# GlassyWing/yolo_deepsort

Measured on AMD Instinct MI355X. Metric: end-to-end frames/sec (detect+ReID+assoc), 608x608, higher is better.
Workload: dtype f16x3

## Files before the change

### yolo_deepsort_amd/csrc/common.h

```cpp
#pragma once
#include <hip/hip_runtime.h>
#include <stdint.h>
#include <stdio.h>
#include <string>
#include <vector>
#include <stdexcept>

namespace yds {

void set_error(const std::string &msg);
struct Error : std::runtime_error {
    explicit Error(const std::string &m) : std::runtime_error(m) {}
};
[[noreturn]] void fail(const char *fmt, ...);
int bound_device();
void bind_thread();
hipStream_t make_stream(bool latency_role);

#define YDS_HIP(expr)                                                                          \
    do {                                                                                       \
        hipError_t _e = (expr);                                                                \
        if (_e != hipSuccess)                                                                  \
            ::yds::fail("%s failed: %s (%s:%d)", #expr, hipGetErrorString(_e), __FILE__, __LINE__); \
    } while (0)

#define YDS_API_BEGIN try { ::yds::bind_thread();
#define YDS_API_END                                                                            \
    }                                                                                          \
    catch (const std::exception &e) {                                                          \
        ::yds::set_error(e.what());                                                            \
        return -1;                                                                             \
    }                                                                                          \
    return 0;
#define YDS_API_END_PTR                                                                        \
    }                                                                                          \
    catch (const std::exception &e) {                                                          \
        ::yds::set_error(e.what());                                                            \
        return nullptr;                                                                        \
    }

template <typename T> struct DevBuf {
    T *p = nullptr;
    size_t n = 0;
    DevBuf() = default;
    explicit DevBuf(size_t count) { alloc(count); }
    DevBuf(const DevBuf &) = delete;
    DevBuf &operator=(const DevBuf &) = delete;
    DevBuf(DevBuf &&o) noexcept : p(o.p), n(o.n) { o.p = nullptr; o.n = 0; }
    DevBuf &operator=(DevBuf &&o) noexcept {
        if (this != &o) { release(); p = o.p; n = o.n; o.p = nullptr; o.n = 0; }
        return *this;
    }
    ~DevBuf() { release(); }
    void alloc(size_t count) {
        release();
        if (count == 0) return;
        YDS_HIP(hipMalloc((void **)&p, count * sizeof(T)));
        n = count;
    }
    void ensure(size_t count) { if (count > n) alloc(count); }
    void release() { if (p) { (void)hipFree(p); p = nullptr; n = 0; } }
    void upload(const T *src, size_t count, hipStream_t s = nullptr) {
        ensure(count);
        if (count) YDS_HIP(hipMemcpyAsync(p, src, count * sizeof(T), hipMemcpyHostToDevice, s));
    }
};

struct View {
    float *p = nullptr;
    int n = 0, h = 0, w = 0, c = 0, ld = 0;
    int fmt = 0;
    size_t pixels() const { return (size_t)n * h * w; }
};

enum Act { ACT_LINEAR = 0, ACT_LEAKY = 1, ACT_MISH = 2, ACT_RELU = 3 };
enum ResMode { RES_NONE = 0, RES_AFTER_ACT = 1, RES_BEFORE_ACT = 2 };

struct ConvArgs {
    View x, y;
    const float *w = nullptr, *bias = nullptr;
    const void *w16 = nullptr;
    View res;
    int ksize = 1, stride = 1, pad = 0, kpad = 0;
    int act = ACT_LINEAR, res_mode = RES_NONE;
    int terms = 3;
    View y2;
    int n_split = 0;
    int tile_gn = 0;
};
enum ConvVariant {
    VAR_F32_128x128_K32, VAR_F32_128x64_K32, VAR_F32_64x64_K32, VAR_F32_128x32_K32, VAR_F32_128x128_K16, VAR_F32_128x64_K16, VAR_F32_64x128_K16,
    VAR_STAGED_128x128, VAR_STAGED_64x128, VAR_STAGED_128x64, VAR_STAGED_64x64,
    VAR_DMA_128x128_NS2, VAR_DMA_256x128_NS3, VAR_DMA_128x256_NS3, VAR_DMA_128x128_NS3, VAR_WIN_256x128, VAR_WIN_256x64, VAR_WIN_128x64,
    VAR_DMA_128x64_NS2, VAR_DMA_64x128_NS2, VAR_WIN2_128x128, VAR_SPLITK_64x128, VAR_SPLITK_128x128, VAR_DIRECT_RGB, kConvVariants
};
static_assert(VAR_STAGED_128x128 == 7 && VAR_WIN_256x128 == 15 && VAR_SPLITK_64x128 == 21 && kConvVariants == 24, "variant ids are fixed");
int launch_conv(const ConvArgs &a, hipStream_t s, int variant = -1);
constexpr int kVariantMask = 0xff, kTileGnShift = 8;
bool conv_presplit_input(const ConvArgs &a);
bool launch_conv_maxpool3s2(const ConvArgs &a, hipStream_t s);
int conv_autotune(const ConvArgs &a, hipStream_t s, float *best_us);
std::vector<int> conv_candidates(const ConvArgs &a);
enum ConvMath { MATH_F32 = 0, MATH_F16X3 = 1 };
int conv_math();
void set_conv_math(int m);
void pack_weights_f16x3(const float *w, int cout, int kpad, std::vector<uint16_t> &out);
const char *conv_variant_name(int v);
double conv_flops(const ConvArgs &a);
double conv_bytes_io(const View &v);
double conv_bytes(const ConvArgs &a);

void launch_maxpool(const View &x, const View &y, int k, int stride, int pad, bool zero_pad_br, hipStream_t s);
void launch_upsample(const View &x, const View &y, int stride, hipStream_t s);
void launch_copy(const View &x, const View &y, hipStream_t s);
void launch_add(const View &a, const View &b, const View &y, hipStream_t s);
void launch_nchw_to_nhwc(const float *src_nchw, const View &y, int c_src, hipStream_t s);
void launch_nhwc_to_nchw(const View &x, float *dst_nchw, hipStream_t s);
void launch_pack_h16(const float *src_f32, const View &y, hipStream_t s);
void launch_yolo_decode(const View &head, float *out, int total_boxes, int box_off, int num_classes,
                        const float *anchors_wh , int A, int img_h, int img_w, hipStream_t s);
void launch_inject(const View &head, int image, const float *rows_dev, int n, int head_index, int num_classes,
                   float logit, hipStream_t s);
void launch_inject_batch(const View &head, int batch, const float *table_dev, const int *offsets_dev, int max_rows, int head_index,
                         int num_classes, float logit, hipStream_t s);
void launch_resize_u8(const uint8_t *frames, int n, int h, int w, const View &y, hipStream_t s, bool bgr = false);
void launch_window_resize(const uint8_t *frames, int h, int w, const int *tiles_dev, int T, int slot0, int n, const View &y, hipStream_t s,
                          bool bgr);
void launch_window_boxes(const float *pred, int n_boxes, int attrs, const int *tiles_dev, const float *scale_dev, int T, int slot0, int n,
                         float *dst, hipStream_t s);
void launch_crop_resize(const uint8_t *frames, int h, int w, const int *boxes5_dev, int D, const View &y,
                        hipStream_t s, bool bgr = false);
void launch_avgpool_l2norm(const View &x, float *out, hipStream_t s);

}
```

### yolo_deepsort_amd/csrc/conv.hip

```cpp
#include "conv_common.h"

#include <vector>

#include <map>
#include <string>
#include <string.h>

namespace yds {

template <int BM, int BN, int WM, int WN, int BK, int ACT, int RES>
__global__ __launch_bounds__(256, 2) void conv_igemm_f32(ConvKernelArgs p) {
    fp16_saturate_on();
    static_assert(WM * WN == 4, "4 waves per workgroup");
    static_assert(BK == 16 || BK == 32, "K step");
    constexpr int LDS_LD = BK + 4;
    constexpr int CPR = BK / 4;
    constexpr int RPP = 256 / CPR;
    constexpr int TM = BM / WM / 32, TN = BN / WN / 32;
    constexpr int A_ROWS = BM / RPP, B_ROWS = BN / RPP;
    static_assert(A_ROWS >= 1 && B_ROWS >= 1, "tile too small for the staging pattern");
    extern __shared__ __attribute__((aligned(16))) float smem[];
    float *As = smem;
    float *Bs = smem + 2 * BM * LDS_LD;

// ... 255 lines not shown
    c.y.h = a.x.h; c.y.w = a.x.w;
    ConvKernelArgs k = make_conv_args(c);
    if (!conv_pool_applicable(k)) return false;
    launch_conv_pool(k, s);
    return true;
}

static int g_math = -1;
int conv_math() {
    if (g_math < 0) {
        const char *e = getenv("YDS_CONV_MATH");
        g_math = (e && !strcmp(e, "f32")) ? MATH_F32 : MATH_F16X3;
    }
    return g_math;
}
void set_conv_math(int m) { g_math = m == MATH_F32 ? MATH_F32 : MATH_F16X3; }

enum ConvArith { ARITH_F32 = MATH_F32, ARITH_F16X3 = MATH_F16X3, ARITH_DIRECT };
struct ConvVariantInfo {
    const char *name;
    int arith;
    void (*launch)(ConvKernelArgs k, int tile, hipStream_t s);
    int tile;
    bool (*runs)(const ConvArgs &a, const ConvKernelArgs &k);
    bool (*timed)(const ConvArgs &a);
};

static void launch_f32(ConvKernelArgs k, int tile, hipStream_t s) {
    switch (tile) {
        case 0: launch_cfg<128, 128, 2, 2, 32>(k, s); break;
        case 1: launch_cfg<128, 64, 2, 2, 32>(k, s); break;
        case 2: launch_cfg<64, 64, 2, 2, 32>(k, s); break;
        case 3: launch_cfg<128, 32, 4, 1, 32>(k, s); break;
        case 4: launch_cfg<128, 128, 2, 2, 16>(k, s); break;
        case 5: launch_cfg<128, 64, 2, 2, 16>(k, s); break;
        default: launch_cfg<64, 128, 2, 2, 16>(k, s); break;
    }
}
static void launch_win2(ConvKernelArgs k, int, hipStream_t s) { launch_conv_win2(k, s); }
static void launch_direct(ConvKernelArgs k, int, hipStream_t s) {
    if (!conv_direct_applicable(k)) fail("conv: the direct RGB kernel does not apply to this layer");
    launch_conv_direct(k, s);
}

static bool runs_not_f16(const ConvArgs &a, const ConvKernelArgs &) { return a.x.fmt != FMT_F16; }
static bool runs_presplit(const ConvArgs &a, const ConvKernelArgs &) { return conv_presplit_input(a); }
static bool runs_win(const ConvArgs &a, const ConvKernelArgs &k) { return conv_presplit_input(a) && conv_win_applicable(k); }
static bool runs_win_small(const ConvArgs &a, const ConvKernelArgs &k) { return runs_win(a, k) && a.terms != 1 && conv_win16_small_applicable(k); }
static bool runs_win2(const ConvArgs &a, const ConvKernelArgs &k) { return conv_presplit_input(a) && conv_win2_applicable(k); }
template <int TILE> static bool runs_splitk(const ConvArgs &a, const ConvKernelArgs &k) { return conv_presplit_input(a) && conv_splitk_applicable(k, TILE); }
static bool runs_direct(const ConvArgs &, const ConvKernelArgs &k) { return conv_direct_applicable(k); }

static bool timed_always(const ConvArgs &) { return true; }
static bool timed_narrow(const ConvArgs &a) { return a.y.c <= 64; }
static bool timed_wide(const ConvArgs &a) { return a.y.c >= 128; }
static bool timed_never(const ConvArgs &) { return false; }
static bool timed_unmerged(const ConvArgs &a) { return !a.n_split; }

static const ConvVariantInfo kVariants[kConvVariants] = {
     {"conv_igemm_f32<128,128,2,2,32>", ARITH_F32, launch_f32, 0, runs_not_f16, timed_always},
     {"conv_igemm_f32<128,64,2,2,32>", ARITH_F32, launch_f32, 1, runs_not_f16, timed_always},
     {"conv_igemm_f32<64,64,2,2,32>", ARITH_F32, launch_f32, 2, runs_not_f16, timed_always},
     {"conv_igemm_f32<128,32,4,1,32>", ARITH_F32, launch_f32, 3, runs_not_f16, timed_narrow},
     {"conv_igemm_f32<128,128,2,2,16>", ARITH_F32, launch_f32, 4, runs_not_f16, timed_always},
     {"conv_igemm_f32<128,64,2,2,16>", ARITH_F32, launch_f32, 5, runs_not_f16, timed_always},
     {"conv_igemm_f32<64,128,2,2,16>", ARITH_F32, launch_f32, 6, runs_not_f16, timed_always},
     {"conv_igemm_f16x3<128,128>", ARITH_F16X3, launch_conv_f16x3_staged, 0, runs_not_f16, timed_always},
     {"conv_igemm_f16x3<64,128>", ARITH_F16X3, launch_conv_f16x3_staged, 1, runs_not_f16, timed_always},
     {"conv_igemm_f16x3<128,64>", ARITH_F16X3, launch_conv_f16x3_staged, 2, runs_not_f16, timed_always},
     {"conv_igemm_f16x3<64,64>", ARITH_F16X3, launch_conv_f16x3_staged, 3, runs_not_f16, timed_always},
     {"conv_igemm_f16x3_dma<128,128,2x2,2>", ARITH_F16X3, launch_conv_f16x3_dma, 0, runs_presplit, timed_always},
     {"conv_igemm_f16x3_dma<256,128,4x2,3>", ARITH_F16X3, launch_conv_f16x3_dma, 1, runs_presplit, timed_always},
     {"conv_igemm_f16x3_dma<128,256,2x4,3>", ARITH_F16X3, launch_conv_f16x3_dma, 2, runs_presplit, timed_always},
     {"conv_igemm_f16x3_dma<128,128,2x2,3>", ARITH_F16X3, launch_conv_f16x3_dma, 3, runs_presplit, timed_always},
     {"conv3x3_f16x3_win<256,128,4x2>", ARITH_F16X3, launch_conv_f16x3_win, 0, runs_win, timed_always},
     {"conv3x3_f16x3_win<256,64,8x1>", ARITH_F16X3, launch_conv_f16x3_win, 1, runs_win, timed_narrow},
     {"conv3x3_f16x3_win<128,64,4x1>", ARITH_F16X3, launch_conv_f16x3_win, 2, runs_win_small, timed_narrow},
     {"conv_igemm_f16x3_dma<128,64,2x2,2>", ARITH_F16X3, launch_conv_f16x3_dma, 4, runs_presplit, timed_always},
     {"conv_igemm_f16x3_dma<64,128,2x2,2>", ARITH_F16X3, launch_conv_f16x3_dma, 5, runs_presplit, timed_always},
     {"conv3x3_f16x3_win2<128,128,2x2>", ARITH_F16X3, launch_win2, 0, runs_win2, timed_wide},
     {"conv_igemm_f16x3_dma<64,128,2x2,2>+splitK", ARITH_F16X3, launch_conv_f16x3_splitk, 0, runs_splitk<0>, timed_never},
     {"conv_igemm_f16x3_dma<128,128,2x2,2>+splitK", ARITH_F16X3, launch_conv_f16x3_splitk, 1, runs_splitk<1>, timed_never},
     {"conv3x3_rgb_direct", ARITH_DIRECT, launch_direct, 0, runs_direct, timed_unmerged},
};

const char *conv_variant_name(int v) {
    if (v >= 0) v &= kVariantMask;
    return v >= 0 && v < kConvVariants ? kVariants[v].name : "?";
}

int launch_conv(const ConvArgs &a, hipStream_t s, int variant) {
    ConvKernelArgs k = make_conv_args(a);
    if (variant >= 0) {
        k.gn_req = std::max(a.tile_gn, (variant >> kTileGnShift) & 0xff);
        variant &= kVariantMask;
    } else {
        k.gn_req = a.tile_gn;
    }
    if (variant < 0 || variant >= kConvVariants) variant = conv_default_variant(a);
    const ConvVariantInfo &e = kVariants[variant];
    if (e.arith == ARITH_F32 && (k.fmt_x != FMT_F32 || k.fmt_y != FMT_F32 || k.fmt_r != FMT_F32))
        fail("conv: the fp32 MFMA kernel takes fp32 tensors only");
    if (e.arith == ARITH_F16X3) {
        if (!a.w16) fail("conv: f16x3 variant requested but the layer has no split weights");
        k.w = reinterpret_cast<const float *>(a.w16);
    }
    e.launch(k, e.tile, s);
    return variant;
}

std::vector<int> conv_candidates(const ConvArgs &a) {
    const ConvKernelArgs k = make_conv_args(a);
    std::vector<int> cand;
    for (int v = 0; v < kConvVariants; ++v) {
        const ConvVariantInfo &e = kVariants[v];
        if ((e.arith == conv_math() || e.arith == ARITH_DIRECT) && e.runs(a, k) && e.timed(a)) cand.push_back(v);
    }
    return cand;
}

static int conv_autotune_measured(const ConvArgs &a, hipStream_t s, float *best_us);

static std::map<std::string, int> &tune_cache() {
    static std::map<std::string, int> cache;
    static bool loaded = false;
    if (!loaded) {
        loaded = true;
        if (const char *path = getenv("YDS_TUNE_CACHE")) {
            if (FILE *f = fopen(path, "r")) {
                char key[256];
                int v;
                while (fscanf(f, "%255s %d", key, &v) == 2) cache[key] = v;
                fclose(f);
            }
        }
    }
    return cache;
}
static std::string tune_key(const ConvArgs &a) {
    char buf[256];
    int n = a.x.n;
    if (n > 64) {
        int p2 = 64;
        while (p2 * 2 <= n) p2 *= 2;
        n = n >= p2 + p2 / 2 ? p2 + p2 / 2 : p2;
    }
    snprintf(buf, sizeof buf, "m%d_n%d_h%d_w%d_c%d_ld%d_o%d_ho%d_wo%d_k%d_s%d_a%d_r%d_fx%d_fy%d_sp%d", conv_math() + (a.terms == 1 ? 10 : 0), n, a.x.h, a.x.w, a.x.c, a.x.ld, a.y.c,
             a.y.h, a.y.w, a.ksize, a.stride, a.act, a.res.p ? a.res_mode : 0, a.x.fmt, a.y.fmt, a.n_split);
    return buf;
}

int conv_autotune(const ConvArgs &a, hipStream_t s, float *best_us) {
    if (getenv("YDS_NO_AUTOTUNE")) return -1;
    if (const char *f = getenv("YDS_CONV_FORCE")) {
        const int v = atoi(f);
        if (v >= 0 && v < kConvVariants && kVariants[v].runs(a, make_conv_args(a))) return v;
        return conv_autotune_measured(a, s, best_us);
    }
    if (conv_math() == MATH_F16X3 && a.w16 && a.terms != 1 && a.n_split == 0 && conv_splitk_preferred(make_conv_args(a))) return VAR_SPLITK_64x128;
    const std::string key = tune_key(a);
    auto &cache = tune_cache();
    auto it = cache.find(key);
    if (it != cache.end()) return it->second;
    int v = conv_autotune_measured(a, s, best_us);
    cache[key] = v;
    if (const char *path = getenv("YDS_TUNE_CACHE")) {
// ... 51 lines not shown
```

### yolo_deepsort_amd/csrc/conv_common.h

```cpp
#pragma once
#include "common.h"
#include "h16.h"

#include <algorithm>
#include <stdlib.h>
#include <type_traits>

namespace yds {

typedef float f32x16 __attribute__((ext_vector_type(16)));
typedef float f32x4 __attribute__((ext_vector_type(4)));

typedef _Float16 h8 __attribute__((ext_vector_type(8)));
typedef _Float16 h4 __attribute__((ext_vector_type(4)));
constexpr float A_SCALE = 1.f / 256.f, LO_SCALE = 2048.f;
typedef __attribute__((address_space(3))) void lds_void_t;
typedef __attribute__((address_space(1))) const void glb_void_t;
template <int N> __device__ __forceinline__ void wait_vmcnt() { asm volatile("s_waitcnt vmcnt(%0)" ::"n"(N) : "memory"); }

struct ConvKernelArgs {
    const float *x, *w, *bias, *res;
    float *y;
    int H, W, Cin, ldx;
    int Ho, Wo, Cout, ldy, ldr;
    int ksize, stride, pad;
    int K, Kpad, M;
    int act, res_mode;
    int fmt_x, fmt_y, fmt_r;
    int terms;
    int ksplit = 1;
    float *y2 = nullptr;
    int ldy2 = 0, n_split = 0;
    int tiles_m, tiles_n, xm, rm, rn;
    int gn = 1;
    int gn_req = 0;
};

constexpr int KALIGN = 32;
constexpr int STAGGER = 24;

template <int ACT> __device__ __forceinline__ float apply_act(float v) {
    if (ACT == ACT_LEAKY) return v > 0.f ? v : v * 0.1f;
    if (ACT == ACT_RELU) return v > 0.f ? v : 0.f;
    if (ACT == ACT_MISH) {
        const float e = __builtin_amdgcn_exp2f(fminf(v, 20.f) * 1.44269504088896341f);
        const float n = e * (e + 2.f);
        const float m = v * (n * __builtin_amdgcn_rcpf(n + 2.f));
        return v > 20.f ? v : m;
    }
    return v;
}

__device__ __forceinline__ bool tile_of_block(const ConvKernelArgs &p, int &tm, int &tn) {
    const int b = blockIdx.x, xcd = b & 7, idx = b >> 3;
    int lm, ln;
    if (p.gn <= 1) {
        lm = idx % p.rm;
        ln = idx / p.rm;
    } else {
        const int per = p.rm * p.gn, grp = idx / per, w = idx - grp * per;
        const int g = min(p.gn, p.rn - grp * p.gn);
        lm = w / g;
        ln = grp * p.gn + (w - lm * g);
    }
    tm = (xcd % p.xm) * p.rm + lm;
    tn = (xcd / p.xm) * p.rn + ln;
    return tm < p.tiles_m && tn < p.tiles_n;
}

inline int plan_tile_map(ConvKernelArgs &k, int BM, int BN) {
    k.tiles_m = (k.M + BM - 1) / BM;
    k.tiles_n = (k.Cout + BN - 1) / BN;
    long best = -1;
    for (int xm = 1; xm <= 8; xm *= 2) {
        int xn = 8 / xm;
        int rm = (k.tiles_m + xm - 1) / xm, rn = (k.tiles_n + xn - 1) / xn;
        long waste = (long)rm * rn * 8 - (long)k.tiles_m * k.tiles_n;
        long cost = ((long)rm * BM + (long)rn * BN) * 64 + waste * (BM + BN);
        if (best < 0 || cost < best) { best = cost; k.xm = xm; k.rm = rm; k.rn = rn; }
    }
    k.gn = std::max(1, std::min(k.gn_req, k.rn));
    return 8 * k.rm * k.rn;
}

struct FlatRows {
    int m0;
    __device__ __forceinline__ int operator()(int row) const { return m0 + row; }
};
template <int BM, int BN, int WM, int WN, int ACT, int RES, int NT, class RowMap, bool ONE_PASS, class Store>
__device__ __forceinline__ void conv_epilogue_core(const ConvKernelArgs &p, Store store, float *stage, RowMap rows, int n0, int tid) {
    constexpr int ROWS = BM / WM, LD = BN + 4, C4 = BN / 4;
    constexpr int RSTEP = NT / C4;
    static_assert(NT % C4 == 0 && C4 % 2 == 0 && ROWS % RSTEP == 0, "tile width must divide the workgroup; lane pairs share a row");
    const int wave = tid >> 6, wm = wave / WN;
    const int c4 = tid % C4, rr = tid / C4;
    const int n = n0 + c4 * 4;
    const bool n_vec = n + 3 < p.Cout;
    const bool second = p.n_split > 0 && n >= p.n_split;
    float *const y_base = second ? p.y2 : p.y;
    const int y_ld = second ? p.ldy2 : p.ldy, ny = second ? n - p.n_split : n;
    float4 bias4 = make_float4(0.f, 0.f, 0.f, 0.f);
    if (n_vec) bias4 = *reinterpret_cast<const float4 *>(p.bias + n);
    else {
        if (n < p.Cout) bias4.x = p.bias[n];
        if (n + 1 < p.Cout) bias4.y = p.bias[n + 1];
        if (n + 2 < p.Cout) bias4.z = p.bias[n + 2];
    }
    constexpr int PER_PASS = ROWS / RSTEP, NRES = RES != RES_NONE ? WM * PER_PASS : 1;
    auto sweep = [&](auto yf_c, auto rf_c) {
        constexpr int YF = decltype(yf_c)::value, RF = decltype(rf_c)::value;
        constexpr bool YH = YF == FMT_H16, RH = RF == FMT_H16, YS = YF == FMT_F16, RS = RF == FMT_F16;
        float4 rraw[NRES];
        if (RES != RES_NONE) {
#pragma unroll
            for (int q = 0; q < NRES; ++q) {
                const int m = rows((q / PER_PASS) * ROWS + rr + (q % PER_PASS) * RSTEP);
                rraw[q] = make_float4(0.f, 0.f, 0.f, 0.f);
                if (m >= 0 && m < p.M && n < p.Cout) {
                    const float *rp = p.res + (size_t)m * p.ldr;
                    if (RH) {
                        const char *g = reinterpret_cast<const char *>(rp + (n & ~31)) + (n & 31) * 2;
                        const float2 hi = *reinterpret_cast<const float2 *>(g), lo = *reinterpret_cast<const float2 *>(g + 64);
                        rraw[q] = make_float4(hi.x, hi.y, lo.x, lo.y);
                    } else if (RS) {
                        const float2 h = *reinterpret_cast<const float2 *>(reinterpret_cast<const char *>(rp) + n * 2);
                        rraw[q] = make_float4(h.x, h.y, 0.f, 0.f);
                    } else if (n_vec) {
                        rraw[q] = *reinterpret_cast<const float4 *>(rp + n);
                    } else {
                        rraw[q].x = rp[n];
                        if (n + 1 < p.Cout) rraw[q].y = rp[n + 1];
                        if (n + 2 < p.Cout) rraw[q].z = rp[n + 2];
                    }
                }
            }
        }
#pragma unroll
        for (int pass = 0; pass < WM; ++pass) {
            if (ONE_PASS ? pass == 0 : wm == pass) store(stage + (ONE_PASS ? wm * ROWS * LD : 0));
            if (!ONE_PASS || pass == 0) __syncthreads();
#pragma unroll
            for (int k2 = 0; k2 < PER_PASS; ++k2) {
                const int r = rr + k2 * RSTEP;
                const int m = rows(pass * ROWS + r);
                const bool live = m >= 0 && m < p.M && n < p.Cout;
                float4 v = *reinterpret_cast<const float4 *>(stage + (ONE_PASS ? pass * ROWS * LD : 0) + r * LD + c4 * 4);
                float rs[4] = {0.f, 0.f, 0.f, 0.f};
                if (RES != RES_NONE) {
                    const float4 t = rraw[RES != RES_NONE ? pass * PER_PASS + k2 : 0];
                    if (RH) {
                        union { float2 f; h16x4 h; } uh, ul;
// ... 170 lines not shown
```

### yolo_deepsort_amd/csrc/conv_f16x3.hip

```cpp
#include "conv_common.h"

#include <map>
#include <mutex>

#include <math.h>
#include <string.h>

namespace yds {


constexpr int ROWB = 144;
__device__ __forceinline__ void split4(const f32x4 &v, h4 &hi, h4 &lo) {
#pragma unroll
    for (int c = 0; c < 4; ++c) {
        float xs = v[c] * A_SCALE;
        _Float16 h = (_Float16)xs;
        hi[c] = h;
        lo[c] = (_Float16)((xs - (float)h) * LO_SCALE);
    }
}

template <int BM, int BN, int ACT, int RES, int AIN>
__global__ __launch_bounds__(256, 2) void conv_igemm_f16x3(ConvKernelArgs p) {
    fp16_saturate_on();
// ... 421 lines not shown
    else for (int k = 0; k < 4; ++k) if (n + k < p.Cout) yp[n + k] = v[k];
}

int conv_splitk_factor(const ConvKernelArgs &k, int BM, int BN) {
    const long tiles = (long)((k.M + BM - 1) / BM) * ((k.Cout + BN - 1) / BN);
    const int nk = k.K / 32;
    int s = (int)((512 + tiles - 1) / tiles);
    s = std::min(s, std::min(16, nk / 4));
    return s >= 2 ? s : 1;
}

static float *splitk_workspace(size_t floats, hipStream_t s) {
    static std::mutex mu;
    static std::map<hipStream_t, DevBuf<float>> bufs;
    std::lock_guard<std::mutex> lock(mu);
    DevBuf<float> &b = bufs[s];
    if (b.n < floats) {
        YDS_HIP(hipStreamSynchronize(s));
        b.alloc(floats + floats / 2);
    }
    return b.p;
}

template <int BM, int BN> static void launch_splitk(const ConvKernelArgs &k, hipStream_t s) {
    if (k.fmt_x != FMT_H16 || k.Cin % 32) fail("conv: the split-K LDS-DMA kernel needs a pre-split (H16) input");
    if ((size_t)k.Cout * 4 > (size_t)ZERO_PAGE_BYTES) fail("conv: %d filters exceed the zero page used as the split-K bias", k.Cout);
    const int ksplit = conv_splitk_factor(k, BM, BN);
    if (ksplit < 2) fail("conv: split-K does not apply (the layer already has enough tiles or too few K steps)");
    const int ldw = (k.Cout + 3) / 4 * 4;
    float *ws = splitk_workspace((size_t)ksplit * k.M * ldw, s);
    ConvKernelArgs part = k;
    part.y = ws; part.ldy = ldw; part.fmt_y = FMT_F32;
    part.bias = reinterpret_cast<const float *>(zero_page_dev());
    part.res = nullptr; part.res_mode = RES_NONE; part.fmt_r = FMT_F32; part.act = ACT_LINEAR;
    part.ksplit = ksplit;
    launch_cfg_dma<BM, BN, 2, 2, 2>(part, s);
    const int c4 = (k.Cout + 3) / 4;
    hipLaunchKernelGGL(splitk_reduce_kernel, dim3(((size_t)k.M * c4 + 255) / 256), dim3(256), 0, s, ws, ksplit, k.M, ldw, k);
    YDS_HIP(hipGetLastError());
}

bool conv_splitk_preferred(const ConvKernelArgs &k) {
    if (k.fmt_x != FMT_H16 || k.Cin % 32) return false;
    const long tiles = (long)((k.M + 63) / 64) * ((k.Cout + 127) / 128);
    return tiles <= 128 && k.K / 32 >= 32 && conv_splitk_factor(k, 64, 128) >= 2;
}

bool conv_splitk_applicable(const ConvKernelArgs &k, int tile) {
    if (k.fmt_x != FMT_H16 || k.Cin % 32) return false;
    return tile == 0 ? conv_splitk_factor(k, 64, 128) >= 2 : conv_splitk_factor(k, 128, 128) >= 2;
}

template <int BM, int BN> static void launch_cfg16(const ConvKernelArgs &k, hipStream_t s) {
    if (k.fmt_x == FMT_F16) fail("conv: the register-staged kernel does not read 2-byte (F16) activations");
    constexpr size_t smem = 2ull * (BM + BN) * ROWB;
    dispatch_act_res(k, [&](auto A, auto R) {
        if (k.fmt_x == FMT_H16) launch_conv_tiles<conv_igemm_f16x3<BM, BN, A, R, FMT_H16>>(k, BM, BN, 1, 256, smem, s);
        else launch_conv_tiles<conv_igemm_f16x3<BM, BN, A, R, FMT_F32>>(k, BM, BN, 1, 256, smem, s);
    });
}

void launch_conv_f16x3_staged(ConvKernelArgs k, int tile, hipStream_t s) {
    switch (tile) {
        case 0: launch_cfg16<128, 128>(k, s); break;
        case 1: launch_cfg16<64, 128>(k, s); break;
        case 2: launch_cfg16<128, 64>(k, s); break;
        default: launch_cfg16<64, 64>(k, s); break;
    }
}

void launch_conv_f16x3_dma(ConvKernelArgs k, int tile, hipStream_t s) {
    switch (tile) {
        case 0: launch_cfg_dma<128, 128, 2, 2, 2>(k, s); break;
        case 1: launch_cfg_dma<256, 128, 4, 2, 3>(k, s); break;
        case 2: launch_cfg_dma<128, 256, 2, 4, 3>(k, s); break;
        case 3: launch_cfg_dma<128, 128, 2, 2, 3>(k, s); break;
        case 4: launch_cfg_dma<128, 64, 2, 2, 2>(k, s); break;
        default: launch_cfg_dma<64, 128, 2, 2, 2>(k, s); break;
    }
}

void launch_conv_f16x3_win(ConvKernelArgs k, int tile, hipStream_t s) {
    if (!conv_win_applicable(k)) fail("conv: the window-resident kernel needs a 3x3 stride-1 layer with a pre-split input and W <= 95 (W <= 318 for 32 input channels)");
    if (k.terms == 1) launch_conv_win(k, tile, s);
    else launch_conv_win16(k, tile, s);
}

void launch_conv_f16x3_splitk(ConvKernelArgs k, int tile, hipStream_t s) {
    if (tile == 0) launch_splitk<64, 128>(k, s);
    else launch_splitk<128, 128>(k, s);
}

void pack_weights_f16x3(const float *w, int cout, int kpad, std::vector<uint16_t> &out) {
    out.assign((size_t)cout * kpad * 2, 0);
    for (int o = 0; o < cout; ++o)
        for (int k = 0; k < kpad; ++k) {
            float x = w[(size_t)o * kpad + k];
            if (!(fabsf(x) < 65504.f)) fail("conv: weight %g does not fit the fp16 split (|w| must be < 65504)", (double)x);
            _Float16 h = (_Float16)x;
            _Float16 l = (_Float16)((x - (float)h) * LO_SCALE);
            size_t base = ((size_t)o * (kpad / 32) + k / 32) * 64;
            uint16_t hb, lb;
            memcpy(&hb, &h, 2);
            memcpy(&lb, &l, 2);
            out[base + (k & 31)] = hb;
            out[base + 32 + (k & 31)] = lb;
        }
}

}
```

### yolo_deepsort_amd/csrc/conv_win16.hip

```cpp
#include "conv_win_common.h"

namespace yds {
namespace {

template <int BM, int BN, int WM, int WN, int ACT, int RES>
__global__ __launch_bounds__(WM * WN * 64, WM * WN == 8 ? 1 : 2) void conv3x3_f16x3_win16(ConvKernelArgs p, int wrows, int nbuf) {
    fp16_saturate_on();
    constexpr int NW = WM * WN, NT = NW * 64;
    static_assert(NW == 8 || NW == 4, "eight waves (one workgroup per CU) or four (two)");
    constexpr int RW = BM / WM, CW = BN / WN;
    constexpr int TM = RW / 16, TN = CW / 16;
    constexpr int HM = TM / 2, HN = TN / 2;
    static_assert(TM % 2 == 0 && TN % 2 == 0, "the wave tile splits into quadrants");
    constexpr int B_STAGE = BN * ROW;
    constexpr int B_INST = BN / (8 * NW);
    extern __shared__ __attribute__((aligned(16))) char smem[];
    const int WB = wrows * ROW;
    char *bring = smem + nbuf * WB;
    const int zoff = nbuf * WB + NSB * B_STAGE;

    const int tid = threadIdx.x;
    const int lane = tid & 63, wave = __builtin_amdgcn_readfirstlane(tid >> 6);
    const int wm = wave / WN, wn = wave % WN;
    int m0, n0;
    {
        int tm, tn;
        if (!tile_of_block(p, tm, tn)) return;
        m0 = tm * BM;
        n0 = tn * BN;
    }
    if (tid < 32) reinterpret_cast<float *>(smem + zoff)[tid] = 0.f;
    const ClockProbe clk(tid);

    const int W = p.W, G = p.Cin / 32;
    const int drow = lane >> 3, dpos = lane & 7;
    const int npieces = wrows / 8;
    unsigned w_off16[B_INST];
#pragma unroll
    for (int b = 0; b < B_INST; ++b) {
        const int row = (b * NW + wave) * 8 + drow;
        w_off16[b] = (unsigned)min(n0 + row, p.Cout - 1) * (unsigned)(p.Kpad / 4) + (unsigned)(dpos ^ ((row >> 1) & 7));
    }
    const char *x_bytes = reinterpret_cast<const char *>(p.x), *w_bytes = reinterpret_cast<const char *>(p.w);
    auto a_piece = [&](int g, int k) {
        const int pc = min(k * NW + wave, npieces - 1);
        const int j = pc * 8 + drow;
        const int f = min(max(m0 - W - 1 + j, 0), p.M - 1);
        const unsigned off16 = (unsigned)f * (unsigned)(p.ldx / 4) + (unsigned)(dpos ^ ((j >> 1) & 7));
        const char *src = x_bytes + (size_t)g * ROW + ((size_t)off16 << 4);
        __builtin_amdgcn_global_load_lds((glb_void_t *)src, (lds_void_t *)(smem + (g & 1) * WB + pc * 8 * ROW), 16, 0, 0);
    };
    auto b_piece = [&](int g, int tap, int stage, int b) {
        const char *src = w_bytes + (size_t)(tap * G + g) * ROW + ((size_t)w_off16[b] << 4);
        __builtin_amdgcn_global_load_lds((glb_void_t *)src, (lds_void_t *)(bring + stage * B_STAGE + (b * NW + wave) * 8 * ROW), 16, 0, 0);
    };

    const int r0 = wm * RW + (lane & 15);
    unsigned okbits[(TM + 2) / 3];
#pragma unroll
    for (int q = 0; q < (TM + 2) / 3; ++q) okbits[q] = 0;
#pragma unroll
    for (int i = 0; i < TM; ++i) okbits[i / 3] |= tap_valid_bits(p, m0 + r0 + i * 16) << (9 * (i % 3));

    f32x4 acc1[TM][TN], acc2[TM][TN];
#pragma unroll
    for (int i = 0; i < TM; ++i)
#pragma unroll
        for (int j = 0; j < TN; ++j)
#pragma unroll
            for (int e = 0; e < 4; ++e) { acc1[i][j][e] = 0.f; acc2[i][j][e] = 0.f; }

    const int swz = (lane >> 1) & 7, kq = lane >> 4;
    const int b_frag = (wn * CW + (lane & 15)) * ROW;
    const int b_hi = b_frag + (kq ^ swz) * 16;

    h8 ah[TM], al[TM], bh[TN], bl[TN];
    int a_hi[TM];
    auto frag_read = [&](const char *bst, int half, int f) {
        if (f < 2 * HM) {
            const int i = half * HM + f / 2;
            const h8 v = *reinterpret_cast<const h8 *>(smem + (f & 1 ? a_hi[i] ^ 64 : a_hi[i]));
            if (f & 1) al[i] = v; else ah[i] = v;
        } else {
            const int g = f - 2 * HM, j = half * HN + g / 2;
            const h8 v = *reinterpret_cast<const h8 *>(bst + j * 16 * ROW + (g & 1 ? b_hi ^ 64 : b_hi));
            if (g & 1) bl[j] = v; else bh[j] = v;
        }
    };
    constexpr int NRH = 2 * (HM + HN);
    constexpr int NMQ = 3 * HM * HN;
    auto mfma = [&](int qa, int qb, int m) {
        const int ij = m % (HM * HN), term = m / (HM * HN), i = qa * HM + ij / HN, j = qb * HN + ij % HN;
        if (term == 0) acc1[i][j] = __builtin_amdgcn_mfma_f32_16x16x32_f16(ah[i], bh[j], acc1[i][j], 0, 0, 0);
        else if (term == 1) acc2[i][j] = __builtin_amdgcn_mfma_f32_16x16x32_f16(ah[i], bl[j], acc2[i][j], 0, 0, 0);
        else acc2[i][j] = __builtin_amdgcn_mfma_f32_16x16x32_f16(al[i], bh[j], acc2[i][j], 0, 0, 0);
    };
    auto tap_addr = [&](int g, int tap) {
        const int shift = (tap / 3) * W + (tap % 3);
        const int wbase = (g & 1) * WB;
        int rj = r0 + shift;
        asm volatile("" : "+v"(rj));
#pragma unroll
        for (int i = 0; i < TM; ++i) {
            const bool ok = (okbits[i / 3] >> (9 * (i % 3) + tap)) & 1u;
            const int j = rj + i * 16;
            a_hi[i] = ok ? wbase + j * ROW + ((kq ^ ((j >> 1) & 7)) << 4) : zoff + (kq << 4);
        }
    };
    auto step = [&](auto tap_c, int g, auto last_c) {
        constexpr int TAP = decltype(tap_c)::value;
        constexpr bool LAST = decltype(last_c)::value;
        constexpr bool REFILL = !(LAST && TAP + 2 > 8);
        constexpr bool NEXT = !(LAST && TAP == 8);
        constexpr int TAP1 = (TAP + 1) % 9, TAP2 = (TAP + 2) % 9;
        const int g1 = TAP + 1 >= 9 ? g + 1 : g, g2 = TAP + 2 >= 9 ? g + 1 : g;
        const char *bst = bring + (TAP % NSB) * B_STAGE, *bst1 = bring + ((TAP + 1) % NSB) * B_STAGE;
        auto dma = [&](int o) {
            if (o == 0) { if (!LAST && TAP < APW) a_piece(g + 1, TAP); }
            else if (o - 1 < B_INST) { if (REFILL) b_piece(g2, TAP2, (TAP + 2) % NSB, o - 1); }
        };
        constexpr int NA = 2 * HM, NB = 2 * HN;
#pragma unroll
        for (int m = 0; m < NMQ; ++m) {
            mfma(0, 0, m);
            __builtin_amdgcn_sched_barrier(0);
            if (m < NB) frag_read(bst, 1, NA + m);
            __builtin_amdgcn_sched_barrier(0);
        }
#pragma unroll
        for (int m = 0; m < NMQ; ++m) {
            mfma(0, 1, m);
            __builtin_amdgcn_sched_barrier(0);
            if (m < NA) frag_read(bst, 1, m);
            __builtin_amdgcn_sched_barrier(0);
        }
        wait_vmcnt<0>();
        __builtin_amdgcn_s_barrier();
        if (NEXT) tap_addr(g1, TAP1);
        __builtin_amdgcn_sched_barrier(0);
#pragma unroll
        for (int m = 0; m < NMQ; ++m) {
            mfma(1, 0, m);
            __builtin_amdgcn_sched_barrier(0);
            if (m <= B_INST) dma(m);
            else if (NEXT && m - 1 - B_INST < NA) frag_read(bst1, 0, m - 1 - B_INST);
            __builtin_amdgcn_sched_barrier(0);
        }
        static_assert(1 + B_INST + NA <= NMQ, "Q10 holds the DMA pieces and the A fragments");
#pragma unroll
        for (int m = 0; m < NMQ; ++m) {
            mfma(1, 1, m);
            __builtin_amdgcn_sched_barrier(0);
            if (NEXT && m < NB) frag_read(bst1, 0, NA + m);
            __builtin_amdgcn_sched_barrier(0);
        }
    };
    auto group = [&](int g, auto last_c) { for_each_tap(step, g, last_c); };

    for (int k = 0; k < (npieces + NW - 1) / NW; ++k) a_piece(0, k);
#pragma unroll
    for (int b = 0; b < B_INST; ++b) b_piece(0, 0, 0, b);
#pragma unroll
    for (int b = 0; b < B_INST; ++b) b_piece(0, 1, 1, b);
    wait_vmcnt<B_INST>();
    __syncthreads();
    tap_addr(0, 0);
#pragma unroll
    for (int f = 0; f < NRH; ++f) frag_read(bring, 0, f);
    __builtin_amdgcn_sched_barrier(0);

    for (int g = 0; g + 1 < G; ++g) group(g, std::false_type{});
    group(G - 1, std::true_type{});

    __syncthreads();
#pragma unroll
    for (int i = 0; i < TM; ++i)
#pragma unroll
        for (int j = 0; j < TN; ++j)
#pragma unroll
            for (int e = 0; e < 4; ++e) acc1[i][j][e] = (acc1[i][j][e] + acc2[i][j][e] * (1.f / LO_SCALE)) * (1.f / A_SCALE);
    conv_epilogue16<BM, BN, WM, WN, ACT, RES, TM, TN, NT, true>(p, acc1, reinterpret_cast<float *>(smem), m0, n0, tid);
    clk.end();
}

template <int BM, int BN, int WM, int WN, int ACT, int RES> void launch_inst_win16(ConvKernelArgs k, hipStream_t s) {
    const int nbuf = win_buffers(k.Cin, 32);
    const WinPlan plan = win_plan(WIN128, BM, BN, WM * WN, k.W, nbuf);
    launch_conv_tiles<conv3x3_f16x3_win16<BM, BN, WM, WN, ACT, RES>>(k, BM, BN, 1, WM * WN * 64, plan.launch_bytes, s, plan.wrows, nbuf);
}

constexpr int SMALL_BM = 128, SMALL_BN = 64, SMALL_NW = 4;

}

void conv_win16_clock(unsigned long long *cycles_ticks, bool reset) { clock_probe_read(cycles_ticks, reset); }

bool conv_win16_small_applicable(const ConvKernelArgs &k) {
    if (!conv_win_applicable(k) || k.Cout > SMALL_BN) return false;
    const WinPlan plan = win_plan(WIN128, SMALL_BM, SMALL_BN, SMALL_NW, k.W, win_buffers(k.Cin, 32));
    return plan.prefetch_fits && plan.launch_bytes <= 80 * 1024;
}

void launch_conv_win16(ConvKernelArgs k, int shape, hipStream_t s) {
    if (shape != 0 && shape != 1 && !conv_win16_small_applicable(k)) fail("conv: the 128x64 window-resident tile needs a 3x3 stride-1 layer with a pre-split input, at most 64 filters and W <= 43");
    dispatch_act_res(k, [&](auto A, auto R) {
        if (shape == 0) launch_inst_win16<256, 128, 4, 2, A, R>(k, s);
        else if (shape == 1) launch_inst_win16<256, 64, 8, 1, A, R>(k, s);
        else launch_inst_win16<SMALL_BM, SMALL_BN, SMALL_NW, 1, A, R>(k, s);
    });
}

}
```

### yolo_deepsort_amd/csrc/conv_win_common.h

```cpp
#pragma once
#include "conv_common.h"

#include <utility>

namespace yds {
namespace {

struct WinGeom {
    int row;
    int nsb;
    int apw;
    constexpr int piece() const { return 1024 / row; }
};
constexpr WinGeom WIN128 = {128, 3, 7};
constexpr WinGeom WIN64 = {64, 4, 6};
constexpr int ROW = WIN128.row, NSB = WIN128.nsb, APW = WIN128.apw;

constexpr int win_buffers(int Cin, int group_channels) { return Cin == group_channels ? 1 : 2; }

struct WinPlan {
    int wrows;
    size_t loop_bytes;
    size_t launch_bytes;
    bool prefetch_fits;
};
constexpr WinPlan win_plan(const WinGeom &g, int BM, int BN, int nw, int W, int nbuf) {
    const int wrows = (BM + 2 * W + 2 + g.piece() - 1) / g.piece() * g.piece();
    const size_t loop_bytes = (size_t)nbuf * wrows * g.row + (size_t)g.nsb * BN * g.row + g.row;
    return {wrows, loop_bytes, std::max(loop_bytes, conv_stage_bytes(BM, BN)), nbuf == 1 || wrows <= g.apw * nw * g.piece()};
}

__device__ __forceinline__ unsigned tap_valid_bits(const ConvKernelArgs &p, int m) {
    unsigned bits = 0;
    if (m < p.M) {
        const int W = p.W, HW = p.H * W;
        const int rem = m % HW, y = rem / W, x = rem - y * W;
#pragma unroll
        for (int t = 0; t < 9; ++t) {
            const int yy = y + t / 3 - 1, xx = x + t % 3 - 1;
            bits |= ((unsigned)yy < (unsigned)p.H && (unsigned)xx < (unsigned)W ? 1u : 0u) << t;
        }
    }
    return bits;
}

template <class Step, int... TAP, class... Args> __device__ __forceinline__ void each_tap(Step &step, std::integer_sequence<int, TAP...>, Args... args) {
    (step(std::integral_constant<int, TAP>{}, args...), ...);
}
template <class Step, class... Args> __device__ __forceinline__ void for_each_tap(Step &step, Args... args) {
    each_tap(step, std::make_integer_sequence<int, 9>{}, args...);
}

#ifdef YDS_CLOCK_PROBE
__device__ unsigned long long yds_clk[2];
struct ClockProbe {
    bool sample;
    unsigned long long c0 = 0, w0 = 0;
    __device__ __forceinline__ explicit ClockProbe(int tid) : sample(tid == 0 && (blockIdx.x & 31) == 0) {
        if (sample) { c0 = __builtin_amdgcn_s_memtime(); w0 = wall_clock64(); }
    }
    __device__ __forceinline__ void end() const {
        if (sample) {
            atomicAdd(&yds_clk[0], __builtin_amdgcn_s_memtime() - c0);
            atomicAdd(&yds_clk[1], wall_clock64() - w0);
        }
    }
};
inline void clock_probe_read(unsigned long long *cycles_ticks, bool reset) {
    YDS_HIP(hipMemcpyFromSymbol(cycles_ticks, HIP_SYMBOL(yds_clk), 2 * sizeof(unsigned long long)));
    if (reset) {
        unsigned long long z[2] = {};
        YDS_HIP(hipMemcpyToSymbol(HIP_SYMBOL(yds_clk), z, sizeof z));
    }
}
#else
struct ClockProbe {
    __device__ __forceinline__ explicit ClockProbe(int) {}
    __device__ __forceinline__ void end() const {}
};
inline void clock_probe_read(unsigned long long *cycles_ticks, bool) { cycles_ticks[0] = cycles_ticks[1] = 0; }
#endif

}
}
```

Before: 1666.

## Add persistent window-resident f16x3 conv variants with cross-tile prefetch

Adds two persistent-kernel variants of the window-resident 3x3 f16x3 convolution. The grid is capped at the CU count and each workgroup loops over its tiles. During the last input-channel group of one tile it prefetches the next tile's first input window and filter stages, so loading overlaps the epilogue and tail latency instead of paying a fresh ramp-up per workgroup. The autotuner can pick these variants, at the cost of higher register pressure, more complex code, and a reuse of LDS for the epilogue that must not collide with in-flight prefetches.

```diff
diff --git a/yolo_deepsort_amd/csrc/common.h b/yolo_deepsort_amd/csrc/common.h
--- a/yolo_deepsort_amd/csrc/common.h
+++ b/yolo_deepsort_amd/csrc/common.h
@@ -92,9 +92,10 @@
     VAR_F32_128x128_K32, VAR_F32_128x64_K32, VAR_F32_64x64_K32, VAR_F32_128x32_K32, VAR_F32_128x128_K16, VAR_F32_128x64_K16, VAR_F32_64x128_K16,
     VAR_STAGED_128x128, VAR_STAGED_64x128, VAR_STAGED_128x64, VAR_STAGED_64x64,
     VAR_DMA_128x128_NS2, VAR_DMA_256x128_NS3, VAR_DMA_128x256_NS3, VAR_DMA_128x128_NS3, VAR_WIN_256x128, VAR_WIN_256x64, VAR_WIN_128x64,
-    VAR_DMA_128x64_NS2, VAR_DMA_64x128_NS2, VAR_WIN2_128x128, VAR_SPLITK_64x128, VAR_SPLITK_128x128, VAR_DIRECT_RGB, kConvVariants
+    VAR_DMA_128x64_NS2, VAR_DMA_64x128_NS2, VAR_WIN2_128x128, VAR_SPLITK_64x128, VAR_SPLITK_128x128, VAR_DIRECT_RGB,
+    VAR_WIN_256x128_PERSIST, VAR_WIN_256x64_PERSIST, kConvVariants
 };
-static_assert(VAR_STAGED_128x128 == 7 && VAR_WIN_256x128 == 15 && VAR_SPLITK_64x128 == 21 && kConvVariants == 24, "variant ids are fixed");
+static_assert(VAR_STAGED_128x128 == 7 && VAR_WIN_256x128 == 15 && VAR_SPLITK_64x128 == 21 && VAR_DIRECT_RGB == 23 && VAR_WIN_256x128_PERSIST == 24 && kConvVariants == 26, "variant ids are fixed");
 int launch_conv(const ConvArgs &a, hipStream_t s, int variant = -1);
 constexpr int kVariantMask = 0xff, kTileGnShift = 8;
 bool conv_presplit_input(const ConvArgs &a);
diff --git a/yolo_deepsort_amd/csrc/conv.hip b/yolo_deepsort_amd/csrc/conv.hip
--- a/yolo_deepsort_amd/csrc/conv.hip
+++ b/yolo_deepsort_amd/csrc/conv.hip
@@ -361,6 +361,8 @@
      {"conv_igemm_f16x3_dma<64,128,2x2,2>+splitK", ARITH_F16X3, launch_conv_f16x3_splitk, 0, runs_splitk<0>, timed_never},
      {"conv_igemm_f16x3_dma<128,128,2x2,2>+splitK", ARITH_F16X3, launch_conv_f16x3_splitk, 1, runs_splitk<1>, timed_never},
      {"conv3x3_rgb_direct", ARITH_DIRECT, launch_direct, 0, runs_direct, timed_unmerged},
+     {"conv3x3_f16x3_win<256,128,4x2>+persist", ARITH_F16X3, launch_conv_f16x3_win, 3, runs_win, timed_always},
+     {"conv3x3_f16x3_win<256,64,8x1>+persist", ARITH_F16X3, launch_conv_f16x3_win, 4, runs_win, timed_narrow},
 };
 
 const char *conv_variant_name(int v) {
diff --git a/yolo_deepsort_amd/csrc/conv_common.h b/yolo_deepsort_amd/csrc/conv_common.h
--- a/yolo_deepsort_amd/csrc/conv_common.h
+++ b/yolo_deepsort_amd/csrc/conv_common.h
@@ -51,8 +51,8 @@
     return v;
 }
 
-__device__ __forceinline__ bool tile_of_block(const ConvKernelArgs &p, int &tm, int &tn) {
-    const int b = blockIdx.x, xcd = b & 7, idx = b >> 3;
+__device__ __forceinline__ bool tile_of_block(const ConvKernelArgs &p, int b, int &tm, int &tn) {
+    const int xcd = b & 7, idx = b >> 3;
     int lm, ln;
     if (p.gn <= 1) {
         lm = idx % p.rm;
@@ -67,6 +67,7 @@
     tn = (xcd / p.xm) * p.rn + ln;
     return tm < p.tiles_m && tn < p.tiles_n;
 }
+__device__ __forceinline__ bool tile_of_block(const ConvKernelArgs &p, int &tm, int &tn) { return tile_of_block(p, (int)blockIdx.x, tm, tn); }
 
 inline int plan_tile_map(ConvKernelArgs &k, int BM, int BN) {
     k.tiles_m = (k.M + BM - 1) / BM;
diff --git a/yolo_deepsort_amd/csrc/conv_f16x3.hip b/yolo_deepsort_amd/csrc/conv_f16x3.hip
--- a/yolo_deepsort_amd/csrc/conv_f16x3.hip
+++ b/yolo_deepsort_amd/csrc/conv_f16x3.hip
@@ -527,7 +527,7 @@
 
 void launch_conv_f16x3_win(ConvKernelArgs k, int tile, hipStream_t s) {
     if (!conv_win_applicable(k)) fail("conv: the window-resident kernel needs a 3x3 stride-1 layer with a pre-split input and W <= 95 (W <= 318 for 32 input channels)");
-    if (k.terms == 1) launch_conv_win(k, tile, s);
+    if (k.terms == 1) launch_conv_win(k, tile >= 3 ? tile - 3 : tile, s);
     else launch_conv_win16(k, tile, s);
 }
 
diff --git a/yolo_deepsort_amd/csrc/conv_win16.hip b/yolo_deepsort_amd/csrc/conv_win16.hip
--- a/yolo_deepsort_amd/csrc/conv_win16.hip
+++ b/yolo_deepsort_amd/csrc/conv_win16.hip
@@ -3,11 +3,13 @@
 namespace yds {
 namespace {
 
-template <int BM, int BN, int WM, int WN, int ACT, int RES>
+template <int BM, int BN, int WM, int WN, int ACT, int RES, bool PERSIST = false>
 __global__ __launch_bounds__(WM * WN * 64, WM * WN == 8 ? 1 : 2) void conv3x3_f16x3_win16(ConvKernelArgs p, int wrows, int nbuf) {
     fp16_saturate_on();
     constexpr int NW = WM * WN, NT = NW * 64;
     static_assert(NW == 8 || NW == 4, "eight waves (one workgroup per CU) or four (two)");
+    static_assert(!PERSIST || NW == 8, "the persistent form is built for the one-workgroup-per-CU shapes");
+    static_assert(9 % NSB == 0, "a tile's step 0 uses ring stage 0 (cross-tile filter prefetch)");
     constexpr int RW = BM / WM, CW = BN / WN;
     constexpr int TM = RW / 16, TN = CW / 16;
     constexpr int HM = TM / 2, HN = TN / 2;
@@ -20,12 +22,20 @@
     const int zoff = nbuf * WB + NSB * B_STAGE;
 
     const int tid = threadIdx.x;
-    const int lane = tid & 63, wave = __builtin_amdgcn_readfirstlane(tid >> 6);
+    const int lane = tid & 63;
+    int wave = __builtin_amdgcn_readfirstlane(tid >> 6);
     const int wm = wave / WN, wn = wave % WN;
     int m0, n0;
+    int vb = blockIdx.x;
+    const int nvb = 8 * p.rm * p.rn;
     {
         int tm, tn;
-        if (!tile_of_block(p, tm, tn)) return;
+        if constexpr (PERSIST) {
+            while (vb < nvb && !tile_of_block(p, vb, tm, tn)) vb += gridDim.x;
+            if (vb >= nvb) return;
+        } else {
+            if (!tile_of_block(p, tm, tn)) return;
+        }
         m0 = tm * BM;
         n0 = tn * BN;
     }
@@ -33,7 +43,7 @@
     const ClockProbe clk(tid);
 
     const int W = p.W, G = p.Cin / 32;
-    const int drow = lane >> 3, dpos = lane & 7;
+    int drow = lane >> 3, dpos = lane & 7;
     const int npieces = wrows / 8;
     unsigned w_off16[B_INST];
 #pragma unroll
@@ -41,21 +51,62 @@
         const int row = (b * NW + wave) * 8 + drow;
         w_off16[b] = (unsigned)min(n0 + row, p.Cout - 1) * (unsigned)(p.Kpad / 4) + (unsigned)(dpos ^ ((row >> 1) & 7));
     }
+    bool has_next = false;
+    int m0n = 0, n0n = 0;
+    auto find_next = [&] {
+        has_next = false;
+        for (int v = vb + gridDim.x; v < nvb; v += gridDim.x) {
+            int tm, tn;
+            if (tile_of_block(p, v, tm, tn)) {
+                vb = v;
+                has_next = true;
+                m0n = tm * BM;
+                n0n = tn * BN;
+                break;
+            }
+        }
+        vb = __builtin_amdgcn_readfirstlane(vb);
+        m0n = __builtin_amdgcn_readfirstlane(m0n);
+        n0n = __builtin_amdgcn_readfirstlane(n0n);
+        has_next = __builtin_amdgcn_readfirstlane((int)has_next) != 0;
+    };
     const char *x_bytes = reinterpret_cast<const char *>(p.x), *w_bytes = reinterpret_cast<const char *>(p.w);
-    auto a_piece = [&](int g, int k) {
+    auto a_piece_of = [&](int mt, int g, int k, int drow, int dpos) {
         const int pc = min(k * NW + wave, npieces - 1);
         const int j = pc * 8 + drow;
-        const int f = min(max(m0 - W - 1 + j, 0), p.M - 1);
+        const int f = min(max(mt - W - 1 + j, 0), p.M - 1);
         const unsigned off16 = (unsigned)f * (unsigned)(p.ldx / 4) + (unsigned)(dpos ^ ((j >> 1) & 7));
         const char *src = x_bytes + (size_t)g * ROW + ((size_t)off16 << 4);
         __builtin_amdgcn_global_load_lds((glb_void_t *)src, (lds_void_t *)(smem + (g & 1) * WB + pc * 8 * ROW), 16, 0, 0);
     };
-    auto b_piece = [&](int g, int tap, int stage, int b) {
-        const char *src = w_bytes + (size_t)(tap * G + g) * ROW + ((size_t)w_off16[b] << 4);
+    auto a_piece = [&](int g, int k) { a_piece_of(m0, g, k, drow, dpos); };
+    auto b_piece_of = [&](const unsigned (&off)[B_INST], int g, int tap, int stage, int b) {
+        const char *src = w_bytes + (size_t)(tap * G + g) * ROW + ((size_t)off[b] << 4);
         __builtin_amdgcn_global_load_lds((glb_void_t *)src, (lds_void_t *)(bring + stage * B_STAGE + (b * NW + wave) * 8 * ROW), 16, 0, 0);
     };
-
-    const int r0 = wm * RW + (lane & 15);
+    auto b_piece = [&](int g, int tap, int stage, int b) { b_piece_of(w_off16, g, tap, stage, b); };
+    auto lane_now = [] {
+        int l;
+        asm volatile("v_mbcnt_lo_u32_b32 %0, -1, 0\n\tv_mbcnt_hi_u32_b32 %0, -1, %0" : "=v"(l));
+        return l;
+    };
+    auto a_piece_next = [&](int k) {
+        int mt = m0n;
+        asm volatile("" : "+s"(mt));
+        const int l = lane_now();
+        a_piece_of(mt, 0, k, l >> 3, l & 7);
+    };
+    auto b_piece_next = [&](int tap, int stage, int b) {
+        int nt = n0n;
+        asm volatile("" : "+s"(nt));
+        const int l = lane_now(), drow = l >> 3, dpos = l & 7;
+        const int row = (b * NW + wave) * 8 + drow;
+        const unsigned off[B_INST] = {(unsigned)min(nt + row, p.Cout - 1) * (unsigned)(p.Kpad / 4) + (unsigned)(dpos ^ ((row >> 1) & 7))};
+        const char *src = w_bytes + (size_t)tap * G * ROW + ((size_t)off[0] << 4);
+        __builtin_amdgcn_global_load_lds((glb_void_t *)src, (lds_void_t *)(bring + stage * B_STAGE + (b * NW + wave) * 8 * ROW), 16, 0, 0);
+    };
+
+    int r0 = wm * RW + (lane & 15);
     unsigned okbits[(TM + 2) / 3];
 #pragma unroll
     for (int q = 0; q < (TM + 2) / 3; ++q) okbits[q] = 0;
@@ -70,9 +121,9 @@
 #pragma unroll
             for (int e = 0; e < 4; ++e) { acc1[i][j][e] = 0.f; acc2[i][j][e] = 0.f; }
 
-    const int swz = (lane >> 1) & 7, kq = lane >> 4;
+    int swz = (lane >> 1) & 7, kq = lane >> 4;
     const int b_frag = (wn * CW + (lane & 15)) * ROW;
-    const int b_hi = b_frag + (kq ^ swz) * 16;
+    int b_hi = b_frag + (kq ^ swz) * 16;
 
     h8 ah[TM], al[TM], bh[TN], bl[TN];
     int a_hi[TM];
@@ -102,7 +153,9 @@
         asm volatile("" : "+v"(rj));
 #pragma unroll
         for (int i = 0; i < TM; ++i) {
-            const bool ok = (okbits[i / 3] >> (9 * (i % 3) + tap)) & 1u;
+            unsigned ob = okbits[i / 3];
+            if constexpr (PERSIST) asm volatile("" : "+v"(ob));
+            const bool ok = (ob >> (9 * (i % 3) + tap)) & 1u;
             const int j = rj + i * 16;
             a_hi[i] = ok ? wbase + j * ROW + ((kq ^ ((j >> 1) & 7)) << 4) : zoff + (kq << 4);
         }
@@ -116,8 +169,13 @@
         const int g1 = TAP + 1 >= 9 ? g + 1 : g, g2 = TAP + 2 >= 9 ? g + 1 : g;
         const char *bst = bring + (TAP % NSB) * B_STAGE, *bst1 = bring + ((TAP + 1) % NSB) * B_STAGE;
         auto dma = [&](int o) {
-            if (o == 0) { if (!LAST && TAP < APW) a_piece(g + 1, TAP); }
-            else if (o - 1 < B_INST) { if (REFILL) b_piece(g2, TAP2, (TAP + 2) % NSB, o - 1); }
+            if (o == 0) {
+                if (!LAST && TAP < APW) a_piece(g + 1, TAP);
+                if constexpr (PERSIST && LAST && TAP < APW) { if (has_next) a_piece_next(TAP); }
+            } else if (o - 1 < B_INST) {
+                if (REFILL) b_piece(g2, TAP2, (TAP + 2) % NSB, o - 1);
+                if constexpr (PERSIST && !REFILL) { if (has_next) b_piece_next(TAP2, (TAP + 2) % NSB, o - 1); }
+            }
         };
         constexpr int NA = 2 * HM, NB = 2 * HN;
 #pragma unroll
@@ -162,6 +220,7 @@
     for (int b = 0; b < B_INST; ++b) b_piece(0, 0, 0, b);
 #pragma unroll
     for (int b = 0; b < B_INST; ++b) b_piece(0, 1, 1, b);
+    if constexpr (PERSIST) find_next();
     wait_vmcnt<B_INST>();
     __syncthreads();
     tap_addr(0, 0);
@@ -169,17 +228,76 @@
     for (int f = 0; f < NRH; ++f) frag_read(bring, 0, f);
     __builtin_amdgcn_sched_barrier(0);
 
-    for (int g = 0; g + 1 < G; ++g) group(g, std::false_type{});
-    group(G - 1, std::true_type{});
-
-    __syncthreads();
-#pragma unroll
-    for (int i = 0; i < TM; ++i)
-#pragma unroll
-        for (int j = 0; j < TN; ++j)
-#pragma unroll
-            for (int e = 0; e < 4; ++e) acc1[i][j][e] = (acc1[i][j][e] + acc2[i][j][e] * (1.f / LO_SCALE)) * (1.f / A_SCALE);
-    conv_epilogue16<BM, BN, WM, WN, ACT, RES, TM, TN, NT, true>(p, acc1, reinterpret_cast<float *>(smem), m0, n0, tid);
+    if constexpr (!PERSIST) {
+        for (int g = 0; g + 1 < G; ++g) group(g, std::false_type{});
+        group(G - 1, std::true_type{});
+
+        __syncthreads();
+#pragma unroll
+        for (int i = 0; i < TM; ++i)
+#pragma unroll
+            for (int j = 0; j < TN; ++j)
+#pragma unroll
+                for (int e = 0; e < 4; ++e) acc1[i][j][e] = (acc1[i][j][e] + acc2[i][j][e] * (1.f / LO_SCALE)) * (1.f / A_SCALE);
+        conv_epilogue16<BM, BN, WM, WN, ACT, RES, TM, TN, NT, true>(p, acc1, reinterpret_cast<float *>(smem), m0, n0, tid);
+    } else {
+        for (;;) {
+            {
+                asm volatile("" : "+s"(wave));
+                const int l = lane_now(), wm_t = wave / WN, wn_t = wave % WN;
+                drow = l >> 3;
+                dpos = l & 7;
+                r0 = wm_t * RW + (l & 15);
+                swz = (l >> 1) & 7;
+                kq = l >> 4;
+                b_hi = (wn_t * CW + (l & 15)) * ROW + (kq ^ swz) * 16;
+            }
+            for (int g = 0; g + 1 < G; ++g) group(g, std::false_type{});
+            group(G - 1, std::true_type{});
+
+            __syncthreads();
+#pragma unroll
+            for (int i = 0; i < TM; ++i)
+#pragma unroll
+                for (int j = 0; j < TN; ++j)
+#pragma unroll
+                    for (int e = 0; e < 4; ++e) acc1[i][j][e] = (acc1[i][j][e] + acc2[i][j][e] * (1.f / LO_SCALE)) * (1.f / A_SCALE);
+            const int tid_e = wave * 64 + lane_now();
+            typedef const __attribute__((address_space(4))) ConvKernelArgs *kernarg_t;
+            kernarg_t pk = (kernarg_t)__builtin_amdgcn_kernarg_segment_ptr();
+            asm volatile("" : "+s"(pk));
+            conv_epilogue16<BM, BN, WM, WN, ACT, RES, TM, TN, NT, false>(*(const ConvKernelArgs *)pk, acc1, reinterpret_cast<float *>(smem + WB), m0, n0, tid_e);
+            if (!has_next) break;
+            m0 = m0n;
+            n0 = n0n;
+#pragma unroll
+            for (int b = 0; b < B_INST; ++b) {
+                const int row = (b * NW + wave) * 8 + drow;
+                w_off16[b] = (unsigned)min(n0 + row, p.Cout - 1) * (unsigned)(p.Kpad / 4) + (unsigned)(dpos ^ ((row >> 1) & 7));
+            }
+            find_next();
+#pragma unroll
+            for (int q = 0; q < (TM + 2) / 3; ++q) okbits[q] = 0;
+#pragma unroll
+            for (int i = 0; i < TM; ++i) {
+                int Ht = p.H, Wt = p.W;
+                asm volatile("" : "+s"(Ht), "+s"(Wt));
+                okbits[i / 3] |= tap_valid_bits(Ht, Wt, p.M, m0 + r0 + i * 16) << (9 * (i % 3));
+            }
+#pragma unroll
+            for (int i = 0; i < TM; ++i)
+#pragma unroll
+                for (int j = 0; j < TN; ++j)
+#pragma unroll
+                    for (int e = 0; e < 4; ++e) { acc1[i][j][e] = 0.f; acc2[i][j][e] = 0.f; }
+            wait_vmcnt<0>();
+            __syncthreads();
+            tap_addr(0, 0);
+#pragma unroll
+            for (int f = 0; f < NRH; ++f) frag_read(bring, 0, f);
+            __builtin_amdgcn_sched_barrier(0);
+        }
+    }
     clk.end();
 }
 
@@ -189,6 +307,41 @@
     launch_conv_tiles<conv3x3_f16x3_win16<BM, BN, WM, WN, ACT, RES>>(k, BM, BN, 1, WM * WN * 64, plan.launch_bytes, s, plan.wrows, nbuf);
 }
 
+bool win16_persist_applies(const ConvKernelArgs &k, const WinPlan &plan, int nbuf, int BM, int BN, int WM) {
+    return nbuf == 2 && (k.Cin / 32) % 2 == 0 && plan.prefetch_fits && (size_t)(BM / WM) * (BN + 4) * sizeof(float) <= (size_t)plan.wrows * ROW;
+}
+
+int win16_persist_grid(int blocks) {
+    static const int cus = [] {
+        int dev = 0, n = 0;
+        YDS_HIP(hipGetDevice(&dev));
+        YDS_HIP(hipDeviceGetAttribute(&n, hipDeviceAttributeMultiprocessorCount, dev));
+        return n;
+    }();
+    int grid = std::max(8, cus / 8 * 8);
+    if (const char *e = getenv("YDS_WIN_PERSIST_GRID")) {
+        const int n = atoi(e);
+        if (n < 8 || n % 8) fail("conv: YDS_WIN_PERSIST_GRID must be a positive multiple of 8 (got '%s')", e);
+        grid = std::min(grid, n);
+    }
+    return std::min(blocks, grid);
+}
+
+template <int BM, int BN, int WM, int WN, int ACT, int RES> void launch_inst_win16_persist(ConvKernelArgs k, hipStream_t s) {
+    const int nbuf = win_buffers(k.Cin, 32);
+    const WinPlan plan = win_plan(WIN128, BM, BN, WM * WN, k.W, nbuf);
+    if (!win16_persist_applies(k, plan, nbuf, BM, BN, WM)) return launch_inst_win16<BM, BN, WM, WN, ACT, RES>(k, s);
+    constexpr auto KERN = conv3x3_f16x3_win16<BM, BN, WM, WN, ACT, RES, true>;
+    static size_t attr_set = 0;
+    if (plan.loop_bytes > attr_set) {
+        YDS_HIP(hipFuncSetAttribute(reinterpret_cast<const void *>(KERN), hipFuncAttributeMaxDynamicSharedMemorySize, (int)plan.loop_bytes));
+        attr_set = plan.loop_bytes;
+    }
+    const int grid = win16_persist_grid(plan_tile_map(k, BM, BN));
+    hipLaunchKernelGGL(KERN, dim3(grid), dim3(WM * WN * 64), plan.loop_bytes, s, k, plan.wrows, nbuf);
+    YDS_HIP(hipGetLastError());
+}
+
 constexpr int SMALL_BM = 128, SMALL_BN = 64, SMALL_NW = 4;
 
 }
@@ -202,11 +355,13 @@
 }
 
 void launch_conv_win16(ConvKernelArgs k, int shape, hipStream_t s) {
-    if (shape != 0 && shape != 1 && !conv_win16_small_applicable(k)) fail("conv: the 128x64 window-resident tile needs a 3x3 stride-1 layer with a pre-split input, at most 64 filters and W <= 43");
+    if (shape == 2 && !conv_win16_small_applicable(k)) fail("conv: the 128x64 window-resident tile needs a 3x3 stride-1 layer with a pre-split input, at most 64 filters and W <= 43");
     dispatch_act_res(k, [&](auto A, auto R) {
         if (shape == 0) launch_inst_win16<256, 128, 4, 2, A, R>(k, s);
         else if (shape == 1) launch_inst_win16<256, 64, 8, 1, A, R>(k, s);
-        else launch_inst_win16<SMALL_BM, SMALL_BN, SMALL_NW, 1, A, R>(k, s);
+        else if (shape == 2) launch_inst_win16<SMALL_BM, SMALL_BN, SMALL_NW, 1, A, R>(k, s);
+        else if (shape == 3) launch_inst_win16_persist<256, 128, 4, 2, A, R>(k, s);
+        else launch_inst_win16_persist<256, 64, 8, 1, A, R>(k, s);
     });
 }
 
diff --git a/yolo_deepsort_amd/csrc/conv_win_common.h b/yolo_deepsort_amd/csrc/conv_win_common.h
--- a/yolo_deepsort_amd/csrc/conv_win_common.h
+++ b/yolo_deepsort_amd/csrc/conv_win_common.h
@@ -30,19 +30,20 @@
     return {wrows, loop_bytes, std::max(loop_bytes, conv_stage_bytes(BM, BN)), nbuf == 1 || wrows <= g.apw * nw * g.piece()};
 }
 
-__device__ __forceinline__ unsigned tap_valid_bits(const ConvKernelArgs &p, int m) {
+__device__ __forceinline__ unsigned tap_valid_bits(int H, int W, int M, int m) {
     unsigned bits = 0;
-    if (m < p.M) {
-        const int W = p.W, HW = p.H * W;
+    if (m < M) {
+        const int HW = H * W;
         const int rem = m % HW, y = rem / W, x = rem - y * W;
 #pragma unroll
         for (int t = 0; t < 9; ++t) {
             const int yy = y + t / 3 - 1, xx = x + t % 3 - 1;
-            bits |= ((unsigned)yy < (unsigned)p.H && (unsigned)xx < (unsigned)W ? 1u : 0u) << t;
+            bits |= ((unsigned)yy < (unsigned)H && (unsigned)xx < (unsigned)W ? 1u : 0u) << t;
         }
     }
     return bits;
 }
+__device__ __forceinline__ unsigned tap_valid_bits(const ConvKernelArgs &p, int m) { return tap_valid_bits(p.H, p.W, p.M, m); }
 
 template <class Step, int... TAP, class... Args> __device__ __forceinline__ void each_tap(Step &step, std::integer_sequence<int, TAP...>, Args... args) {
     (step(std::integral_constant<int, TAP>{}, args...), ...);
```

Result: no change. 1661 (-0.3%).
